# xiph/LPCNet

Measured on AMD Instinct MI355X. Metric: 16 kHz samples/sec & concurrent real-time streams, 1/2/4/8 MI355X, higher is better.
Workload: dtype f32; 1 GPU; 2048 concurrent streams (each with its own feature file) per GPU x 25 frames (4000 samples) per step, fp32 weights, register-resident block-sparse GRU-A, bit-exact (PARITY) arithmetic; eight streams per CU as two groups of four half a step apart (BASELINE config 2's 1024 streams fill half of these stream slots: `also.config2_1024_streams`); arithmetic=parity, gru_a_blocks=1382, gru_a_densities=0.05,0.05,0.2 (benchmark model), gru_a_items_per_lane=30, streams_per_gpu=2048, streams_per_workgroup=8

## Files before the change

include/lpcnet.h:

```cpp
#ifndef LPCNET_H_
#define LPCNET_H_

#ifdef __cplusplus
extern "C" {
#endif

#ifndef LPCNET_EXPORT
# if defined(__GNUC__)
#  define LPCNET_EXPORT __attribute__ ((visibility ("default")))
# else
#  define LPCNET_EXPORT
# endif
#endif

#define NB_FEATURES 20
#define NB_TOTAL_FEATURES 36
#define LPCNET_COMPRESSED_SIZE 8
#define LPCNET_PACKET_SAMPLES (4*160)
#define LPCNET_FRAME_SIZE (160)

typedef struct LPCNetState LPCNetState;
typedef struct LPCNetDecState LPCNetDecState;

LPCNET_EXPORT int lpcnet_decoder_get_size(void);
// ... 7 lines not shown
LPCNET_EXPORT int lpcnet_init(LPCNetState *st);
LPCNET_EXPORT LPCNetState *lpcnet_create(void);
LPCNET_EXPORT void lpcnet_destroy(LPCNetState *st);
LPCNET_EXPORT void lpcnet_synthesize(LPCNetState *st, const float *features, short *output, int N);
LPCNET_EXPORT int lpcnet_load_model(LPCNetState *st, const unsigned char *data, int len);

#define LPCNET_HIP_STATE_BYTES 8724

LPCNET_EXPORT void lpcnet_reset_signal(LPCNetState *lpcnet);
LPCNET_EXPORT void run_frame_network(LPCNetState *lpcnet, float *gru_a_condition, float *gru_b_condition,
                                     float *lpc, const float *features);
LPCNET_EXPORT void run_frame_network_deferred(LPCNetState *lpcnet, const float *features);
LPCNET_EXPORT void run_frame_network_flush(LPCNetState *lpcnet);
LPCNET_EXPORT void lpcnet_synthesize_tail_impl(LPCNetState *lpcnet, short *output, int N, int preload);
LPCNET_EXPORT void lpcnet_synthesize_impl(LPCNetState *lpcnet, const float *features, short *output, int N,
                                          int preload);

LPCNET_EXPORT const char *lpcnet_hip_last_error(void);
#define LPCNET_HIP_E_NODEVICE (-2)
#define LPCNET_HIP_E_DEVICE   (-3)
#define LPCNET_HIP_E_ARG      (-4)
#define LPCNET_HIP_E_MODEL    (-5)
LPCNET_EXPORT int lpcnet_hip_status(void);
LPCNET_EXPORT void lpcnet_hip_clear_error(void);
LPCNET_EXPORT int lpcnet_hip_model_status(const LPCNetState *st, int clear);
LPCNET_EXPORT int lpcnet_hip_dispatch_stats(unsigned long long *out3, int reset);
LPCNET_EXPORT const char *lpcnet_hip_build_info(void);
LPCNET_EXPORT void lpcnet_hip_set_codebooks(const float *cb1, const float *cb2, const float *cb3, const float *cb_diff4);
LPCNET_EXPORT int lpcnet_hip_set_default_model(const unsigned char *data, int len);
LPCNET_EXPORT int lpcnet_hip_decoder_load_model(LPCNetDecState *st, const unsigned char *data, int len);
LPCNET_EXPORT int lpcnet_hip_set_device(int device);
LPCNET_EXPORT int lpcnet_hip_check_model(const unsigned char *data, int len, int *info);
LPCNET_EXPORT int lpcnet_hip_x3_image_info(const unsigned char *data, int len, int *desc, int *rows, int *selftest);
LPCNET_EXPORT void lpcnet_hip_shutdown(void);

#ifdef __cplusplus
}
#endif
#endif
```

lpcnet_amd/api.py:

```python
from __future__ import annotations

import ctypes as C
import os

import numpy as np

_HERE = os.path.dirname(os.path.abspath(__file__))
LIB_PATH = os.environ.get("LPCNET_HIP_LIB") or os.path.join(_HERE, "liblpcnet_hip.so")

NB_FEATURES = 20
NB_TOTAL_FEATURES = 36
LPCNET_FRAME_SIZE = 160
LPCNET_COMPRESSED_SIZE = 8
LPCNET_PACKET_SAMPLES = 640

_f32p = np.ctypeslib.ndpointer(np.float32, flags="C_CONTIGUOUS")
_i16p = np.ctypeslib.ndpointer(np.int16, flags="C_CONTIGUOUS")
_u8p = np.ctypeslib.ndpointer(np.uint8, flags="C_CONTIGUOUS")

_lib = None


class LPCNetError(RuntimeError):
    pass
# ... 114 lines not shown
    L.lpcnet_batch_plc_enable.argtypes = [vp, C.c_int]
    L.lpcnet_batch_plc_flavour.argtypes = [vp]
    L.lpcnet_batch_plc_reset.argtypes = [vp, C.c_int, C.c_int]
    L.lpcnet_batch_plc_step.argtypes = [vp, _i16p, _u8p]
    L.lpcnet_batch_plc_step_device.argtypes = [vp, vp, _u8p, vp]
    L.lpcnet_batch_plc_step_device_shard.argtypes = [vp, C.c_int, vp, _u8p, vp]
    L.lpcnet_batch_plc_fec_add.argtypes = [vp, C.c_int, vp]
    L.lpcnet_batch_plc_fec_clear.argtypes = [vp, C.c_int]
    L.lpcnet_batch_plc_fec_feed.argtypes = [vp, vp, vp, vp, vp, vp]
    L.lpcnet_batch_plc_fec_feed_device.argtypes = [vp, vp, vp, vp, vp, vp, vp]
    L.lpcnet_batch_plc_fec_feed_device_shard.argtypes = [vp, C.c_int, vp, vp, vp, vp, vp, vp]
    L.lpcnet_hip_plc_fec_feed_plan.argtypes = [C.c_int, vp, vp, vp, vp, vp, vp]
    L.lpcnet_batch_get_plc_state.argtypes = [vp, C.c_int, vp]
    L.lpcnet_batch_set_plc_state.argtypes = [vp, C.c_int, vp]
    L.lpcnet_batch_plc_burg.argtypes = [vp, _f32p, _f32p]
    L.lpcnet_batch_plc_pred.argtypes = [vp, _f32p, _f32p]
    L.lpcnet_hip_plc_plan.argtypes = [C.c_int, C.c_int, vp, _u8p, vp, vp]
    L.lpcnet_hip_plc_model_info.argtypes = [C.c_char_p, C.c_int, C.POINTER(C.c_int)]
    L.lpcnet_batch_encode.argtypes = [vp, _i16p, _u8p, C.c_int]
    L.lpcnet_batch_encode_device.argtypes = [vp, vp, vp, C.c_int, vp]
    L.lpcnet_batch_encode_device_shard.argtypes = [vp, C.c_int, vp, vp, C.c_int, vp]
    L.lpcnet_batch_compute_features.argtypes = [vp, _i16p, _f32p, C.c_int, C.c_int]
    L.lpcnet_batch_compute_features_device.argtypes = [vp, vp, vp, C.c_int, C.c_int, vp]
    L.lpcnet_batch_encoder_enable.argtypes = [vp, C.c_int]
    L.lpcnet_batch_get_encoder_vq_mem.argtypes = [vp, C.c_int, _f32p]
    L.lpcnet_batch_set_encoder_vq_mem.argtypes = [vp, C.c_int, _f32p]
    L.lpcnet_batch_export_state.argtypes = [vp, C.c_int, vp]
    L.lpcnet_batch_import_state.argtypes = [vp, C.c_int, vp]
    L.lpcnet_batch_set_streams_per_workgroup.argtypes = [vp, C.c_int]
    L.lpcnet_batch_get_streams_per_workgroup.argtypes = [vp]
    L.lpcnet_batch_set_twelve_waves.argtypes = [vp, C.c_int]
    L.lpcnet_batch_get_twelve_waves.argtypes = [vp]
    L.lpcnet_hip_x3_image_info.argtypes = [C.c_char_p, C.c_int, C.POINTER(C.c_int), C.POINTER(C.c_int), C.POINTER(C.c_int)]
    L.lpcnet_batch_tune.argtypes = [vp]
    L.lpcnet_batch_enable_timing.argtypes = [vp, C.c_int]
    L.lpcnet_batch_last_timing.argtypes = [vp, C.POINTER(C.c_float), C.POINTER(C.c_float)]
    L.lpcnet_batch_last_error.restype = C.c_char_p
    L.lpcnet_batch_run_tail.argtypes = [vp, _f32p, _f32p, _f32p, _i16p, C.c_int, C.c_int]
    L.lpcnet_batch_run_frames.argtypes = [vp, _f32p, C.c_int, vp, vp, vp, C.c_int]
    L.lpcnet_batch_state_size.restype = C.c_int
    L.lpcnet_batch_get_raw_state.argtypes = [vp, C.c_int, vp]
    L.lpcnet_batch_set_raw_state.argtypes = [vp, C.c_int, vp]
    L.lpcnet_batch_debug_trace.argtypes = [vp, C.c_int, vp]
    L.lpcnet_batch_profile.argtypes = [vp, vp]
    _u32p = np.ctypeslib.ndpointer(np.uint32, flags="C_CONTIGUOUS")
    L.lpcnet_hip_arith_identities_device.argtypes = [_f32p, _f32p, _u32p, _u32p, _u32p, _u32p, C.c_int]
    L.lpcnet_hip_quant_sweep_device.argtypes = [C.POINTER(C.c_ulonglong)]
    L.lpcnet_hip_status.restype = C.c_int
    L.lpcnet_hip_clear_error.restype = None
    L.lpcnet_hip_model_status.argtypes = [vp, C.c_int]
    L.lpcnet_hip_build_info.restype = C.c_char_p
    L.lpcnet_hip_dispatch_stats.argtypes = [C.POINTER(C.c_ulonglong), C.c_int]
    _lib = L
    return L


def check_model(blob: bytes):
    info = (C.c_int * 6)()
    rc = load_library().lpcnet_hip_check_model(blob, len(blob), info)
    return rc, list(info)


def plc_model_info(blob: bytes):
    info = (C.c_int * 7)()
    if load_library().lpcnet_hip_plc_model_info(blob, len(blob), info) != 0:
        raise LPCNetError("plc_model_info: " + last_error())
    return dict(zip(("present", "servable", "d1", "g1", "g2", "nb1", "nb2"), list(info)))


def x3_image_info(blob: bytes):
    desc, rows, st = (C.c_int * (12 * 5 * 4))(), (C.c_int * (12 * 5 * 64))(), C.c_int(-1)
    have = load_library().lpcnet_hip_x3_image_info(blob, len(blob), desc, rows, C.byref(st))
    return have, np.array(desc, np.int32).reshape(12, 5, 4), np.array(rows, np.int32).reshape(12, 5, 64), st.value


def last_error() -> str:
    return load_library().lpcnet_hip_last_error().decode()


def status() -> int:
    return load_library().lpcnet_hip_status()


def clear_error() -> None:
    load_library().lpcnet_hip_clear_error()


def build_info() -> dict:
    txt = load_library().lpcnet_hip_build_info().decode()
    return dict(kv.split("=", 1) for kv in txt.split())


def dispatch_stats(reset=False):
    out = (C.c_ulonglong * 3)()
    load_library().lpcnet_hip_dispatch_stats(out, 1 if reset else 0)
    return int(out[0]), int(out[1]), int(out[2])


def quant_sweep():
    out = (C.c_ulonglong * 3)()
    rc = load_library().lpcnet_hip_quant_sweep_device(out)
    if rc:
        raise LPCNetError(f"lpcnet_hip_quant_sweep_device failed ({rc}): " + last_error())
    return int(out[0]), int(out[1]), int(out[2])


def arith_identities(a: np.ndarray, b: np.ndarray):
    a = np.ascontiguousarray(a, np.float32); b = np.ascontiguousarray(b, np.float32)
# ... 447 lines not shown
```

lpcnet_amd/csrc/api.c:

```c
#include <pthread.h>
#include <math.h>
#include <stddef.h>
#include <stdio.h>
#include <stdlib.h>
#include <string.h>
#include "lpcnet.h"
#include "lpcnet_batch.h"
#include "lpcnet_engine.h"

#define LPCN_MAGIC 0x4C50434Eu

#define MAX_FEATURE_BUFFER_SIZE 4

struct LPCNetState {
    uint32_t magic;
    int32_t model_id;
    lpcn_stream_state s;
    float gru_a_condition[LPCN_ROWS_A];
    float gru_b_condition[LPCN_ROWS_B];
    float feature_buffer[NB_FEATURES * MAX_FEATURE_BUFFER_SIZE];
    int32_t feature_buffer_fill;
};

_Static_assert(sizeof(struct LPCNetState) == LPCNET_HIP_STATE_BYTES, "include/lpcnet.h: LPCNET_HIP_STATE_BYTES is stale");
// ... 1497 lines not shown
        if (pf < 0) st = 100;
        else if (pf == 0) {
            f.pk_b_w = m.pk_b_w; f.pk_b_wq = m.pk_b_wq; f.pk_b_start = m.pk_b_start; f.pk_b_blk = m.pk_b_blk;
            const int sf = lpcn_model_selftest(&f);
            if (sf) st = 100 + sf;
            f.pk_b_w = NULL; f.pk_b_wq = NULL; f.pk_b_start = NULL; f.pk_b_blk = NULL;
            lpcn_model_release(&f);
        }
    }
    if (!st && !m.is_int8) {
        lpcn_model_host f;
        if (lpcn_model_pack_x2(&m, &f) == 0) {
            f.pk_b_w = m.pk_b_w; f.pk_b_start = m.pk_b_start; f.pk_b_blk = m.pk_b_blk;
            const int sf = lpcn_model_selftest(&f);
            if (sf) st = 200 + sf;
            f.pk_b_w = NULL; f.pk_b_start = NULL; f.pk_b_blk = NULL;
            lpcn_model_release(&f);
        }
    }
    if (!st) {
        lpcn_x3_image im;
        if (lpcn_model_pack_x3(&m, &im) == 0) {
            const int sf = lpcn_x3_image_selftest(&m, &im);
            if (sf) st = 300 + sf;
            lpcn_x3_image_release(&im);
        }
    }
    if (info) { info[0] = m.is_int8; info[1] = m.nb_a; info[2] = m.nb_b; info[3] = m.nw; info[4] = m.nb_b_padded; info[5] = st; }
    lpcn_model_release(&m);
    if (st) { set_err("internal error: device packing inconsistent with blob"); return -1; }
    return 0;
}

int lpcnet_hip_x3_image_info(const unsigned char *data, int len, int *desc, int *rows, int *selftest)
{
    lpcn_model_host m;
    lpcn_x3_image im;
    if (lpcn_model_parse(&m, data, len) != 0) { set_err("malformed or incomplete DNNw weight blob"); return -1; }
    const int have = lpcn_model_pack_x3(&m, &im) == 0;
    if (have) {
        if (selftest) *selftest = lpcn_x3_image_selftest(&m, &im);
        for (int w = 0; w < LPCN_X3_WAVES; w++)
            for (int k = 0; k <= LPCN_X3_SEGS; k++) {
                int *d = desc ? desc + (w * (1 + LPCN_X3_SEGS) + k) * 4 : NULL;
                if (d) { d[0] = im.kind[w][k]; d[1] = im.first[w][k]; d[2] = im.count[w][k]; d[3] = im.skip[w][k]; }
                if (rows) memcpy(rows + (w * (1 + LPCN_X3_SEGS) + k) * 64, im.row[w][k], sizeof(int) * 64);
            }
        lpcn_x3_image_release(&im);
    }
    lpcn_model_release(&m);
    return have;
}
```

lpcnet_amd/csrc/engine.hip:

```cpp
#include <hip/hip_runtime.h>
#include <stdio.h>
#include <stdlib.h>
#include <string.h>
#include <memory>
#include <vector>
#include "lpcnet_engine.h"
#include "lpcnet_tables_gen.h"
#include "sample_variants.h"
#include "sample_kernel.hip.h"
#include "frame_kernels.hip.h"
#include "decode_kernel.hip.h"
#include "analysis_kernels.hip.h"
#include "encode_kernels.hip.h"
#include "plc_kernels.hip.h"
#include "plc_plan.h"
#include <math.h>

static thread_local char g_err[512] = "";
extern "C" const char *lpcn_last_error(void) { return g_err; }

#define HIP_TRY(expr)                                                                         \
    do {                                                                                      \
        hipError_t _e = (expr);                                                               \
        if (_e != hipSuccess) {                                                               \
// ... 339 lines not shown
    UP(float, b_bias, m->b_bias, 2 * LPCN_ROWS_B);
    UP(float, fc_w, m->fc_w, 256 * 2 * LPCN_N_B);
    UP(float, fc_b, m->fc_b, 512);
    UP(float, fc_f, m->fc_f, 512);
    {
        std::vector<uint32_t> wh(256 * 2 * LPCN_N_B / 2);
        for (size_t i = 0; i < wh.size(); ++i) {
            const _Float16 lo = (_Float16)m->fc_w[2 * i], hi = (_Float16)m->fc_w[2 * i + 1];
            uint16_t l, h;
            memcpy(&l, &lo, 2); memcpy(&h, &hi, 2);
            wh[i] = (uint32_t)l | ((uint32_t)h << 16);
        }
        UP(uint32_t, fc_wh, wh.data(), wh.size());
    }
    UP(float, tab_tansig, lpcn_tansig, 201);
    UP(float, tab_ulaw2lin, lpcn_ulaw2lin_tab, 256);
    UP(float, tab_logit, lpcn_logit_tab, 256);
#undef UP
    a.nb_b = m->nb_b_padded;
    a.b_dense = m->b_dense;
    if (!m->is_int8 && m->b_dense && !getenv("LPCNET_HIP_NO_X2_IMAGE")) {
        lpcn_model_host mx;
        if (lpcn_model_pack_x2(m, &mx) == 0) {
            const int nwx = round_up_variant(variants_x2, mx.nw);
            mx.pk_b_w = m->pk_b_w; mx.pk_b_start = m->pk_b_start; mx.pk_b_blk = m->pk_b_blk;
            const int stx = lpcn_model_selftest(&mx);
            mx.pk_b_w = nullptr; mx.pk_b_start = nullptr; mx.pk_b_blk = nullptr;
            if (nwx && stx == 0) {
                LpcnSampleArgs &ax = e->image[IMG_X2].args;
                rc = upload_gru_a(&mx, e->image[IMG_X2], nwx);
                if (!rc) rc = upload<float>(e, &ax.emb_nat_sig, m->emb_sig, (size_t)256 * LPCN_ROWS_A);
                if (!rc) rc = upload<float>(e, &ax.emb_nat_pred, m->emb_pred, (size_t)256 * LPCN_ROWS_A);
                if (!rc) rc = upload<float>(e, &ax.emb_nat_exc, m->emb_exc, (size_t)256 * LPCN_ROWS_A);
            }
            lpcn_model_release(&mx);
            if (rc) return fail(rc);
        }
        lpcn_x3_image im;
        if (e->image[IMG_X2].present && lpcn_model_pack_x3(m, &im) == 0) {
            if (lpcn_x3_image_selftest(m, &im) == 0) {
                GruAImage &img = e->image[IMG_X3];
                LpcnSampleArgs &ax = img.args;
                ax = e->image[IMG_X2].args;
                int bound[LPCN_X3_WAVES * (1 + LPCN_X3_SEGS)], head[LPCN_X3_WAVES];
                for (int wv = 0; wv < LPCN_X3_WAVES; ++wv) {
                    int end = 0;
                    bound[wv * (1 + LPCN_X3_SEGS)] = 0;
                    for (int k = 1; k <= LPCN_X3_SEGS; ++k) {
                        if (im.kind[wv][k] != LPCN_X3_NONE) end = im.first[wv][k] + im.count[wv][k];
                        bound[wv * (1 + LPCN_X3_SEGS) + k] = end;
                    }
                    head[wv] = im.kind[wv][0] != LPCN_X3_NONE ? im.count[wv][0] : 0;
                }
                const float *dw = nullptr;
                rc = upload<float>(e, &dw, im.w, (size_t)LPCN_X3_WAVES * LPCN_X3_NW * 64 * 4);
                ax.a_w = (const float4 *)dw;
                if (!rc) rc = upload<uint8_t>(e, &ax.a_blk, im.blk, (size_t)LPCN_X3_WAVES * LPCN_X3_NW * 64);
                if (!rc) rc = upload<int>(e, &ax.a_row, &im.row[0][0][0], (size_t)LPCN_X3_WAVES * (1 + LPCN_X3_SEGS) * 64);
                if (!rc) rc = upload<int>(e, &ax.a_bound, bound, LPCN_X3_WAVES * (1 + LPCN_X3_SEGS));
                if (!rc) rc = upload<int>(e, &ax.a_head, head, LPCN_X3_WAVES);
                img.nw_variant = LPCN_X3_NW; img.present = rc == 0;
            }
            lpcn_x3_image_release(&im);
            if (rc) return fail(rc);
        }
    }
// ... 1466 lines not shown
```

lpcnet_amd/csrc/lpcnet_engine.h:

```cpp
#ifndef LPCNET_ENGINE_H
#define LPCNET_ENGINE_H

#include <stddef.h>
#include <stdint.h>

#ifdef __cplusplus
extern "C" {
#endif

#define LPCN_N_A        384
#define LPCN_N_B        16
#define LPCN_COND       128
#define LPCN_NB_FEAT    20
#define LPCN_PITCH_EMB  64
#define LPCN_FRAME_IN   (LPCN_NB_FEAT + LPCN_PITCH_EMB)
#define LPCN_LPC_ORDER  16
#define LPCN_NB_BANDS   18
#define LPCN_FRAME_SIZE 160
#define LPCN_FEATURES_DELAY 2
#define LPCN_ROWS_A     (3 * LPCN_N_A)
#define LPCN_ROWS_B     (3 * LPCN_N_B)

#define LPCN_WG_THREADS 512
#define LPCN_WAVES      8
#define LPCN_MAX_SLOTS  3
#define LPCN_EARLY_MAX  24
#define LPCN_DEAL_EH_F32 24
#define LPCN_DEAL_HW_I8 3
#define LPCN_I8_GBWA 2
#define LPCN_I8_GBWB 3
#define LPCN_DEAL_HMASK_I8 (0xFFu & ~((1u << LPCN_I8_GBWA) | (1u << LPCN_I8_GBWB)))
#define LPCN_DEAL_EH_I8 22
#define LPCN_X2_CHAIN_WAVES 4
#define LPCN_X2_P0_FIRST 4
#define LPCN_X2_NW_MAX 32
#define LPCN_X3_WAVES 12
#define LPCN_X3_THREADS (64 * LPCN_X3_WAVES)
#define LPCN_X3_CHAIN_WAVES 4
#define LPCN_X3_NW 16
#define LPCN_X3_SEGS 4
#define LPCN_X3_LW 4
#define LPCN_X3_FREE 9
#define LPCN_DEAL_EH_FAST_I8 0

#define LPCN_PLC_IN       (2 * LPCN_NB_BANDS + LPCN_NB_FEAT + 1)
#define LPCN_PLC_MAX_UNITS 512
#define LPCN_PLC_MAX_FEC   100
#define LPCN_PLC_BUF_SIZE  (LPCN_FEATURES_DELAY * LPCN_FRAME_SIZE + 80)
#define LPCN_PLC_QUEUE     (LPCN_PLC_BUF_SIZE + LPCN_FRAME_SIZE)
#define LPCN_PLC_FBUF      4
typedef struct lpcn_plc_model {
    int present;
    int d1, g1, g2;
    int nb1, nb2;
    const float *dense1_w, *dense1_b;
    const float *gru1_w, *gru1_rec, *gru1_bias;
    const int *gru1_idx;
    const float *gru2_w, *gru2_rec, *gru2_bias;
    const int *gru2_idx;
    const float *out_w, *out_b;
} lpcn_plc_model;

typedef struct lpcn_model_host {
    int is_int8;
    int b_dense;
    int nb_a, nb_b;
    int nw;
    int nb_b_padded;
    float lpc_gamma;

    const float *emb_sig, *emb_pred, *emb_exc;
    const float *a_dense_w, *a_dense_b;
    const float *b_dense_w, *b_dense_b;
    const float *conv1_w, *conv1_b, *conv2_w, *conv2_b;
    const float *pitch_emb;
    const float *dense1_w, *dense1_b, *dense2_w, *dense2_b;
    const float *fc_w, *fc_b, *fc_f;
    const float *a_bias, *a_diag;
    const float *a_w; const int *a_idx;
    const float *b_bias;
    const float *b_w; const int *b_idx;
    const float *b_rec;

    float   *pk_a_w;
    int32_t *pk_a_wq;
    int32_t *pk_b_wq;
    uint8_t *pk_a_blk;
    int32_t *pk_a_row;
    int32_t  pk_a_bound[LPCN_WAVES][LPCN_MAX_SLOTS + 1];
    int32_t  pk_a_allh[LPCN_WAVES][LPCN_MAX_SLOTS];
    int32_t  pk_a_head[LPCN_WAVES];
    float   *pk_b_w;
    int32_t *pk_b_start;
    uint8_t *pk_b_blk;
    float   *pk_emb[3];
    lpcn_plc_model plc;
} lpcn_model_host;

enum { LPCN_X3_NONE = 0, LPCN_X3_WHOLE = 1, LPCN_X3_HEAD = 2, LPCN_X3_TAIL = 3 };
typedef struct lpcn_x3_image {
    float   *w;
    uint8_t *blk;
    int32_t  row[LPCN_X3_WAVES][1 + LPCN_X3_SEGS][64];
    int32_t  kind[LPCN_X3_WAVES][1 + LPCN_X3_SEGS];
    int32_t  first[LPCN_X3_WAVES][1 + LPCN_X3_SEGS];
    int32_t  count[LPCN_X3_WAVES][1 + LPCN_X3_SEGS];
    int32_t  skip[LPCN_X3_WAVES][1 + LPCN_X3_SEGS];
} lpcn_x3_image;

int  lpcn_model_parse(lpcn_model_host *m, const unsigned char *blob, int len);
void lpcn_model_release(lpcn_model_host *m);
int  lpcn_model_pack_x2(const lpcn_model_host *m, lpcn_model_host *f);
int  lpcn_model_pack_fast(const lpcn_model_host *m, lpcn_model_host *f);
int  lpcn_model_pack_x3(const lpcn_model_host *m, lpcn_x3_image *im);
void lpcn_x3_image_release(lpcn_x3_image *im);
int  lpcn_x3_image_selftest(const lpcn_model_host *m, const lpcn_x3_image *im);
int  lpcn_model_selftest(const lpcn_model_host *m);
int  lpcn_plc_servable(const lpcn_model_host *m);
void lpcn_plc_pack_rec_i8(const signed char *rec, int N, int32_t *out);

typedef struct lpcn_stream_state {
    float gru_a[LPCN_N_A];
    float gru_b[LPCN_N_B];
    float conv1_mem[2 * LPCN_FRAME_IN];
// ... 152 lines not shown
```

lpcnet_amd/csrc/model_pack.c:

```c
#include <stdio.h>
#include <stdlib.h>
#include <string.h>
#include "lpcnet_engine.h"

typedef struct { const char *name; int size; const void *data; } blob_rec;

static int blob_walk(const unsigned char *p, int len, blob_rec *out, int cap)
{
    int n = 0;
    while (len > 0) {
        int32_t h[5];
        if (len < 64) return -1;
        memcpy(h, p, sizeof(h));
        if (h[3] <= 0 || h[4] < h[3] || h[4] > len - 64) return -1;
        if (h[4] & 3) return -1;
        if (p[63] != 0) return -1;
        if (n == cap) return -1;
        out[n].name = (const char *)(p + 20);
        out[n].size = h[3];
        out[n].data = p + 64;
        n++;
        p += 64 + h[4];
        len -= 64 + h[4];
    }
// ... 103 lines not shown
                }
                if (pick < 0) { ok = 0; break; }
                d.items[pick] += slot_max[z]; d.nsl[pick]++; d.nzr[pick]++; d.zr_items[pick] += slot_max[z];
                trial[z] = pick;
            }
            if (ok) {
                long mx = 0, sum = 0;
                for (int w = 0; w < LPCN_WAVES; w++) { const long c = deal_wave_cost(dp, &d, w); if (c > mx) mx = c; sum += c; }
                if (best_max < 0 || mx < best_max || (mx == best_max && sum < best_sum)) {
                    best_max = mx; best_sum = sum;
                    memcpy(best_wave, trial, sizeof(int) * (size_t)ns);
                }
            }
            depth--;
            if (depth < 0) break;
            used[perm[depth]] = 0;
        }
        int w = perm[depth] + 1;
        while (w < LPCN_WAVES && used[w]) w++;
        if (w >= LPCN_WAVES) {
            perm[depth] = -1;
            depth--;
            if (depth < 0) break;
            used[perm[depth]] = 0;
            continue;
        }
        perm[depth] = w; used[w] = 1;
        depth++;
        if (depth < nc) perm[depth] = -1;
    }
    if (best_max < 0) return -1;
    memcpy(wave_of, best_wave, sizeof(int) * (size_t)ns);
    return 0;
}

static int pack_gru_a(lpcn_model_host *m, int for_fast)
{
    deal_params dpv, *const dp = &dpv;
    enum { NG = LPCN_ROWS_A / 8, NSLOT = NG / 8 };
    row_group g[NG];
    const int *idx = m->a_idx;
    int blk = 0;
    for (int i = 0; i < NG; i++) {
        g[i].group = i; g[i].count = *idx++; g[i].pos = idx; g[i].first_block = blk;
        idx += g[i].count; blk += g[i].count;
    }
    const char *old_i8 = getenv("LPCN_DEAL_I8_OLD");
    const int deal2 = !m->is_int8 || !(old_i8 && old_i8[0] == '1');
    {
        const char *eh = getenv("LPCN_DEAL_EH");
        dp->eh = (eh && *eh) ? atoi(eh) : (m->is_int8 ? LPCN_DEAL_EH_I8 : LPCN_DEAL_EH_F32);
        {
            const char *hw = getenv("LPCN_DEAL_HW");
            dp->hw = (hw && *hw) ? atoi(hw) : (m->is_int8 ? LPCN_DEAL_HW_I8 : LPCN_WAVES / 2);
            if (dp->hw < 2) dp->hw = 2;
            if (dp->hw > LPCN_WAVES / 2) dp->hw = LPCN_WAVES / 2;
            if (!m->is_int8) dp->hw = LPCN_WAVES / 2;
            dp->hmask = (0xFFu << dp->hw) & 0xFFu;
            const char *hm = getenv("LPCN_DEAL_HMASK");
            if (m->is_int8 && !for_fast && !(hw && *hw)) dp->hmask = LPCN_DEAL_HMASK_I8;
            if (m->is_int8 && hm && *hm) dp->hmask = (unsigned)strtoul(hm, NULL, 0) & 0xFFu;
        }
        if (for_fast == 1) {
            const char *ehf = getenv("LPCN_DEAL_EH_FAST");
            dp->eh = (ehf && *ehf) ? atoi(ehf) : LPCN_DEAL_EH_FAST_I8;
        }
// ... 143 lines not shown
        int cur = 0;
        for (int k = 0; k < LPCN_MAX_SLOTS; k++) {
            const int s = slot_at[w][k], j0 = cur;
            const int head = (k == 0) ? m->pk_a_head[w] : 0;
            m->pk_a_bound[w][k] = j0;
            m->pk_a_allh[w][k] = 1;
            if (s < 0) continue;
            int allh = 1;
            for (int q = 0; q < 8; q++) {
                const row_group *rg = &g[8 * s + q];
                if (rg->group * 8 < 2 * LPCN_N_A) allh = 0;
                for (int r = 0; r < 8; r++) {
                    int lane = 8 * q + r;
                    m->pk_a_row[(w * LPCN_MAX_SLOTS + k) * 64 + lane] = rg->group * 8 + r;
                    for (int j = 0; j < rg->count; j++) {
                        const int pos = j < head ? nw - head + j : j0 + (j - head);
                        size_t item = ((size_t)w * nw + pos) * 64 + lane;
                        if (m->is_int8) {
                            const signed char *blkq = (const signed char *)m->a_w + (size_t)(rg->first_block + j) * 32;
                            memcpy(&m->pk_a_wq[item], blkq + r * 4, 4);
                        } else {
                            const float *blkw = m->a_w + (size_t)(rg->first_block + j) * 32;
                            for (int c = 0; c < 4; c++) m->pk_a_w[item * 4 + c] = blkw[c * 8 + r];
                        }
                        m->pk_a_blk[item] = (uint8_t)(rg->pos[j] >> 2);
                    }
                }
            }
            m->pk_a_allh[w][k] = allh;
            cur += slot_max[s] - head;
        }
        m->pk_a_bound[w][LPCN_MAX_SLOTS] = cur;
    }
    if (for_fast == 2) return 0;
    const float *src[3] = {m->emb_sig, m->emb_pred, m->emb_exc};
    for (int tb = 0; tb < 3; tb++) {
        float *dst = (float *)calloc((size_t)256 * LPCN_MAX_SLOTS * LPCN_WG_THREADS, sizeof(float));
        if (!dst) return -1;
        for (int v = 0; v < 256; v++)
            for (int w = 0; w < LPCN_WAVES; w++)
                for (int lane = 0; lane < 64; lane++)
                    for (int k = 0; k < LPCN_MAX_SLOTS; k++) {
                        int r = m->pk_a_row[(w * LPCN_MAX_SLOTS + k) * 64 + lane];
                        dst[((size_t)v * LPCN_MAX_SLOTS + k) * LPCN_WG_THREADS + w * 64 + lane] = r >= 0 ? src[tb][(size_t)v * LPCN_ROWS_A + r] : 0.f;
                    }
        m->pk_emb[tb] = dst;
    }
    return 0;
}

static int pack_gru_b(lpcn_model_host *m)
{
    enum { NG = LPCN_ROWS_B / 8 };
    const size_t cap = (size_t)m->nb_b + 3 * NG + 8;
    if (m->is_int8) m->pk_b_wq = (int32_t *)calloc(8 * cap, sizeof(int32_t));
    else            m->pk_b_w = (float *)calloc(32 * cap, sizeof(float));
    m->pk_b_blk = (uint8_t *)calloc(cap, 1);
    m->pk_b_start = (int32_t *)malloc(sizeof(int32_t) * (NG + 1));
    if ((!m->pk_b_w && !m->pk_b_wq) || !m->pk_b_blk || !m->pk_b_start) return -1;
    const int *idx = m->b_idx;
    int src_blk = 0, dst = 0, dense = 1;
    for (int g = 0; g < NG; g++) {
        int cnt = *idx++;
        m->pk_b_start[g] = dst;
        if (cnt != LPCN_N_A / 4) dense = 0;
        for (int j = 0; j < cnt; j++, src_blk++, dst++) {
            if (m->is_int8) {
// ... 475 lines not shown
```

lpcnet_amd/csrc/sample_kernel.hip.h:

```cpp
#pragma once
#include <hip/hip_runtime.h>
#include <stdint.h>
#include <type_traits>
#include "lpcnet_engine.h"
#include "lpcnet_math.h"

struct LpcnSampleArgs {
    const float *emb_sig, *emb_pred, *emb_exc;
    const float4 *a_w;
    const uint8_t *a_blk;
    const int *a_row;
    const int *a_bound;
    const int *a_allh;
    const int *a_head;
    const float *a_bias1;
    const float *a_diag;
    const float *b_w;
    const int *b_start;
    const uint8_t *b_blk;
    const float *b_rec;
    const float *b_bias;
    const float *fc_w, *fc_b, *fc_f;
    const float *tab_tansig, *tab_ulaw2lin, *tab_logit;
    int nb_b;
    int b_dense;
    int n_streams, n_frames, preload, fc_advance;
    int frame_len;
    const float *cond_a;
    const float *cond_b;
    const float *lpc;
    const int *fc_base;
    short *pcm;
    long long pcm_stride;
    lpcn_stream_state *state;
    float *dbg;
    unsigned long long *prof;
    const uint32_t *fc_wh;
    int fc_f16;
    const float *emb_nat_sig, *emb_nat_pred, *emb_nat_exc;
};

#ifndef LPCN_ENABLE_PROF
#define LPCN_ENABLE_PROF 0
#endif
#define LPCN_DBG_STRIDE 1600

#include "sample_common.hip.h"
#include "quant_i8.hip.h"

namespace lpcn {

#define LPCN_PROD_BLOCKS 48
template <int S> struct Lds {
    static constexpr int HA_STRIDE = 16 * S;
    static constexpr int hA     = 0;
    static constexpr int hA_sz  = 96 * HA_STRIDE + 24 * 16;
    static constexpr int pre    = hA + hA_sz;
    static constexpr int inh    = pre + S * RA * 4;
    static constexpr int cond   = inh + S * NA * 4;
    static constexpr int abias  = cond + S * RA * 4;
    static constexpr int adiag  = abias + RA * 4;
    static constexpr int hT     = adiag + RA * 4;
    static constexpr int hB     = hT + NA * S * 4;
    static constexpr int idx    = hB + S * NB * 4;
    static constexpr int thr    = idx + S * 16;
    static constexpr int mask   = thr + S * 32;
    static constexpr int lead   = mask + S * 64;
    static constexpr int flag   = lead + S * 32;
    static constexpr int condb  = flag + 16;
    static constexpr int lpc    = condb + S * RB * 4;
    static constexpr int sig    = lpc + S * 64;
    static constexpr int pcmbuf = sig + S * 64;
// ... 1291 lines not shown
```

lpcnet_amd/csrc/sample_kernel_x2.hip.h:

```cpp
#pragma once
#include "sample_kernel.hip.h"
#include "tree_stages.h"

namespace lpcn {

#define LPCN_X2_LW 4
#define LPCN_X2_TW 0
#define LPCN_X2_S2W 7
#define LPCN_X2_S2_LEAD 2
#define LPCN_X2_HG 10

struct LdsX2 {
    static constexpr int S = 4;
    static constexpr int HA_STRIDE = 16 * S;
    static constexpr int g_hA    = 0;
    static constexpr int g_hT    = g_hA + 96 * HA_STRIDE + 24 * 16;
    static constexpr int g_prec  = g_hT + NA * S * 4;
    static constexpr int g_hB    = g_prec + NA * S * 4;
    static constexpr int g_idx   = g_hB + S * NB * 4;
    static constexpr int g_thr   = g_idx + S * 16;
    static constexpr int g_mask  = g_thr + S * 32;
    static constexpr int g_pfx   = g_mask + S * 4;
    static constexpr int g_lead  = g_mask + S * 64;
    static constexpr int g_flag  = g_lead + S * 32;
    static constexpr int g_condb = g_flag + 16;
    static constexpr int g_lpc   = g_condb + S * RB * 4;
    static constexpr int g_pcm   = g_lpc + S * 64;
    static constexpr int G_SZ    = g_pcm + S * 320;
    static constexpr int pre_ur  = 2 * G_SZ;
    static constexpr int inh     = pre_ur + 2 * NA * S * 4;
    static constexpr int abias   = inh + NA * S * 4;
    static constexpr int tansig  = abias + 2 * RA * 4;
    static constexpr int ulaw    = tansig + 816;
    static constexpr int logit   = ulaw + 1024;
    static constexpr int brec    = logit + 1024;
    static constexpr int bbias   = brec + NB * RB * 4;
    static constexpr int bstart  = bbias + 2 * RB * 4;
    static constexpr int bw      = bstart + 32;
    static constexpr int total(int nb_b) { return bw + (nb_b + 8) * 128; }
    __host__ __device__ static constexpr int ha_off(int p) { return p * HA_STRIDE + (p >> 2) * 16; }
};

typedef float tree_f4 __attribute__((ext_vector_type(4)));
struct TreeRow { tree_f4 w[NB / 4]; float bias, factor; };
__device__ __forceinline__ TreeRow tree_row_load_node(const LPCN_GLOBAL float *fc_w, const LPCN_GLOBAL float *fc_b, const LPCN_GLOBAL float *fc_f, const int node, const int chan)
{
    const auto *wp = (const LPCN_GLOBAL tree_f4 *)(fc_w + (node * 2 + chan) * NB);
    TreeRow r;
#pragma unroll
    for (int j = 0; j < NB / 4; ++j) r.w[j] = wp[j];
    r.bias = fc_b[chan * 256 + node];
    r.factor = fc_f[chan * 256 + node];
    return r;
}
template <int STAGE>
__device__ __forceinline__ TreeRow tree_row_load(const LPCN_GLOBAL float *fc_w, const LPCN_GLOBAL float *fc_b, const LPCN_GLOBAL float *fc_f, const int lane, const int prefix)
{
    return tree_row_load_node(fc_w, fc_b, fc_f, lpcn_tree_node(STAGE, lpcn_tree_lane_local(STAGE, lane), prefix), lane & 1);
}
__device__ __forceinline__ TreeRow tree_row_load_packed(const LPCN_GLOBAL float *fc_w, const LPCN_GLOBAL float *fc_b, const LPCN_GLOBAL float *fc_f, const int lane, const int prefix)
{
    return tree_row_load_node(fc_w, fc_b, fc_f, lpcn_tree_packed_node(lane, prefix), lane & 1);
}
__device__ __forceinline__ unsigned long long tree_node_ballot(const TreeRow &r, const float *h_s, const float *thr, const float *tansig)
{
    const float4 *hp = (const float4 *)h_s;
    float sum = r.bias;
#pragma unroll
    for (int j = 0; j < NB / 4; ++j) {
        const float4 hv = hp[j];
        const tree_f4 wv = r.w[j];
// ... 49 lines not shown
        const int lane = tid0 & 63, wave = tid0 >> 6;
        const size_t base = (size_t)wave * NW * 64 + lane;
        const int lane_sel = (lane & 3) * 16;
        const auto *ab = as_global(Ap->a_blk);
        const auto *aw = (const LPCN_GLOBAL float *)as_global(Ap->a_w);
#pragma unroll
        for (int j = 0; j < NW; ++j) {
            const auto *v = aw + (base + (size_t)j * 64) * 4;
            w[j] = make_float4(v[0], v[1], v[2], v[3]);
        }
#pragma unroll
        for (int j = 0; j < NW; j += 2) {
            const int p0 = ab[base + (size_t)j * 64];
            const int p1 = (j + 1 < NW) ? ab[base + (size_t)(j + 1) * 64] : 0;
            offp[j >> 1] = (uint32_t)(L::ha_off(p0) + lane_sel) | ((uint32_t)(L::ha_off(p1) + lane_sel) << 16);
        }
        const auto *ar = as_global(Ap->a_row);
#pragma unroll
        for (int k = 0; k < 3; ++k) row_reg[k] = ar[(wave * 3 + k) * 64 + lane];
    }
    int b1 = __builtin_amdgcn_readfirstlane(as_global(Ap->a_bound)[(tid0 >> 6) * 4 + 1]);
    int b2 = __builtin_amdgcn_readfirstlane(as_global(Ap->a_bound)[(tid0 >> 6) * 4 + 2]);
    int b3 = __builtin_amdgcn_readfirstlane(as_global(Ap->a_bound)[(tid0 >> 6) * 4 + 3]);
    const bool allh0 = __builtin_amdgcn_readfirstlane(as_global(Ap->a_allh)[(tid0 >> 6) * 3]) != 0;
    const LPCN_GLOBAL float *fc_w_s = as_global(Ap->fc_w), *fc_b_s = as_global(Ap->fc_b), *fc_f_s = as_global(Ap->fc_f);
    asm volatile("" : "+s"(fc_w_s), "+s"(fc_b_s), "+s"(fc_f_s));
    const LPCN_GLOBAL float *cond_a_s = as_global(Ap->cond_a);
    asm volatile("" : "+s"(cond_a_s));
    const int has_slot = __builtin_amdgcn_readfirstlane((__ballot(row_reg[0] >= 0) != 0ull ? 1 : 0) | (__ballot(row_reg[1] >= 0) != 0ull ? 2 : 0) |
                                                        (__ballot(row_reg[2] >= 0) != 0ull ? 4 : 0));
    const bool has2 = (has_slot & 4) != 0;
    const int hl = __builtin_amdgcn_readfirstlane(as_global(Ap->a_head)[tid0 >> 6]);
    const bool early_wave = hl > 0;
    const bool plain_start = __builtin_amdgcn_readfirstlane(((early_wave || __ballot(row_reg[0] >= 2 * NA) == 0ull) && __ballot(row_reg[1] >= 2 * NA || row_reg[2] >= 2 * NA) == 0ull) ? 1 : 0) != 0;

    {
        const int tid = tid0;
        stage_tables<L>(smem, Ap, tid, NB * RB);
        stage_grub_weights(smem + L::bw, Ap, tid, true);
        for (int i = tid; i < 2 * S * NA; i += LPCN_WG_THREADS) {
            const int gs = i / NA, n = i % NA, g = gs >> 2, s = gs & 3;
            const float hv0 = states[stream_of(gs)].gru_a[n];
            unsigned char *gb = smem + g * L::G_SZ;
            ((float *)(gb + L::g_hT))[n * S + s] = hv0;
            *(float *)(gb + L::g_hA + L::ha_off(n >> 2) + s * 16 + (n & 3) * 4) = hv0;
        }
        for (int i = tid; i < 2 * S * NB; i += LPCN_WG_THREADS) {
            const int gs = i / NB, g = gs >> 2, s = gs & 3;
            ((float *)(smem + g * L::G_SZ + L::g_hB))[s * NB + i % NB] = states[stream_of(gs)].gru_b[i % NB];
        }
        if (tid < 2 * S) {
            const int g = tid >> 2, s = tid & 3;
            unsigned char *gb = smem + g * L::G_SZ;
            stage_leader_record({(float *)(gb + L::g_lead), (int *)(gb + L::g_idx), nullptr, nullptr}, s, &states[stream_of(tid)]);
        }
        if (tid < 2) { int *fl = (int *)(smem + tid * L::G_SZ + L::g_flag); fl[0] = 0; fl[1] = 0; }
        if (tid < 2 * S) ((int *)(smem + (tid >> 2) * L::G_SZ + L::g_pfx))[tid & 3] = 0;
    }
    __syncthreads();

    const bool is_lw = (tid0 >> 6) == LW;
    const bool is_tw_lane = tid0 >= 64 * TW && tid0 < 64 * TW + S;
#define LPCN_LROW ((tid0 & 63) >> 4)
#define LPCN_TAP (tid0 & 15)
    float histP = is_lw ? states[stream_of(S + LPCN_LROW)].last_sig[LPCN_TAP] : 0.f;
    float histQ = is_lw ? states[stream_of(LPCN_LROW)].last_sig[LPCN_TAP] : 0.f;
    bool liveP = false, liveQ = false;
    int live_maskP = 0, live_maskQ = 0;
    int seqP = 0, seqQ = 0;
    int smpP = 0, smpQ = 0, fP = 0, fQ = 0;
    float lpc_tap = 0.f, prod_old = 0.f;

    const int T = n_frames * frame_len;
#if LPCN_ENABLE_PROF
#ifndef LPCN_PROF_MASK
#define LPCN_PROF_MASK 0xFFF
#endif
    unsigned long long *const prof = Ap->prof;
    unsigned long long pt[12] = {0, 0, 0, 0, 0, 0, 0, 0, 0, 0, 0, 0}, tprev = 0;
    const bool profiling = prof != nullptr && blockIdx.x == 0;
#define LPCN_X2_PROF(slot) do { if (((LPCN_PROF_MASK >> (slot)) & 1) && profiling) { const unsigned long long now_ = __builtin_amdgcn_s_memtime(); pt[slot] += now_ - tprev; tprev = now_; } } while (0)
    if (profiling) tprev = __builtin_amdgcn_s_memtime();
#else
#define LPCN_X2_PROF(slot) do { } while (0)
#endif
    for (int h = -1; h <= 2 * T + 1; ++h) {
        const int p = h & 1, q = p ^ 1;
        unsigned char *const gp = smem + p * L::G_SZ, *const gq = smem + q * L::G_SZ;
        const bool p_active = h >= 0 && (h >> 1) < T;
        const bool p_prev = h >= 2;
// ... 253 lines not shown
                LPCN_REMAT_V(r);
                if (r >= 0) {
                    float *c = pre_cell(r, gq);
#pragma unroll
                    for (int s = 0; s < S; ++s) c[s] = acc[s];
                }
            }
            if (p0_wave) { reduce(3, 0); if (fifth) reduce(4, 1); }
            LPCN_X2_PROF(3);
        }

        static_assert(LPCN_X2_S2W > LPCN_X2_LW && LPCN_X2_S2W < LPCN_WAVES && LPCN_TREE_FIELDS == S && LPCN_X2_S2_LEAD >= 1, "stage 2 runs on a row wave other than the leader's, one field per stream");
        const bool s2_wave = q_chain && wave == LPCN_X2_S2W;
        TreeRow sub = {};
        int pfx = 0;
        auto s2_open = [&]() __attribute__((always_inline)) {
            int t_ = tid0;
            LPCN_REMAT_V(t_);
            const uint32_t cell = lds_addr(gq + L::g_pfx) + (uint32_t)lpcn_tree_packed_field(t_ & 63) * 4u;
            do {
                asm volatile("ds_read_b32 %0, %1\n\ts_waitcnt lgkmcnt(0)" : "=v"(pfx) : "v"(cell) : "memory");
            } while (__ballot((pfx >> LPCN_TREE_TOP) != seqQ) != 0ull);
            pfx &= (1 << LPCN_TREE_TOP) - 1;
            sub = tree_row_load_packed(fc_w_s, fc_b_s, fc_f_s, t_ & 63, pfx);
        };
        const bool s2_in_items = s2_wave && p_active && b3 > 0;
        if (s2_wave && !s2_in_items) s2_open();

        if (p_active) {
            hA_cur = gp + L::g_hA;
            load_negz();
            lds_poll_until<false>(p0cnt_p, seqP * NP0);
            LPCN_X2_PROF(11);
            if (plain_start) {
                int r = LPCN_ROW(0);
                LPCN_REMAT_V(r);
                r = r < 0 ? 0 : r;
                const float *c = pre_cell(r, gp);
#pragma unroll
                for (int s = 0; s < S; ++s) acc[s] = c[s];
            } else {
#pragma unroll
            for (int k = 0; k < 3; ++k) {
                int r = LPCN_ROW(k);
                LPCN_REMAT_V(r);
                const bool live_row = r >= 0;
                r = r < 0 ? 0 : r;
                const bool candidate = r >= 2 * NA;
                const int n = candidate ? r - 2 * NA : 0;
                const float bias = sm_abias[2 * r], diag = sm_abias[2 * r + 1];
                float *c = pre_cell(r, gp);
                const bool parked = k == 0 && early_wave;
#pragma unroll
                for (int s = 0; s < S; ++s) {
                    const float bv = bias + diag * hT_p[n * S + s];
                    if (k == 0) acc[s] = (candidate && !parked) ? bv : c[s];
                    else if (candidate && live_row) c[s] = bv;
                }
            }
            }
            auto row_swap = [&](const int k_done, const int k_next) __attribute__((always_inline)) {
                int r = LPCN_ROW(k_done), r2 = LPCN_ROW(k_next);
                LPCN_REMAT_V(r);
                LPCN_REMAT_V(r2);
                if (r >= 0) {
                    float *c = pre_cell(r, gp);
#pragma unroll
// ... 29 lines not shown
                if (j + PF < NW) fetch_h(j + PF);
                if (__builtin_expect(j == nextb, 0)) {
                    if (j == b1) row_swap(0, 1);
                    if (j == b2) row_swap(1, 2);
                    if (j == s2_at) s2_open();
                    __builtin_amdgcn_s_waitcnt(0xC07F);
                    nextb = b1 > j ? b1 : (b2 > j ? b2 : NW);
                    if (s2_at > j && s2_at < nextb) nextb = s2_at;
                }
                mac(j);
                return true;
            };
            auto run_items = [&](auto self, auto jc) __attribute__((always_inline)) -> void {
                constexpr int j = decltype(jc)::value;
                if constexpr (j < NW) {
                    if (!item(j)) return;
                    self(self, std::integral_constant<int, j + 1>{});
                }
            };
            run_items(run_items, std::integral_constant<int, 0>{});
            LPCN_X2_PROF(5);
            if (b1 >= jend) {
                row_swap(0, 1);
                row_swap(1, 2);
                row_store(2);
            } else if (b2 >= jend) {
                row_swap(1, 2);
                row_store(2);
            } else {
                row_store(2);
            }
            LPCN_X2_PROF(6);
        }
        if (s2_wave) {
            int t_ = tid0;
            LPCN_REMAT_V(t_);
            const int ln = t_ & 63, f = lpcn_tree_packed_field(ln);
            const unsigned long long m = tree_node_ballot(sub, hB_q + f * NB, (const float *)(gq + L::g_thr) + f * 8 + lpcn_tree_packed_level(ln), sm_tansig) & lpcn_tree_packed_mask();
            int walks = 0;
#pragma unroll
            for (int k = 0; k < S; ++k) walks |= lpcn_tree_packed_walk(m, k) << (8 * k);
            if ((ln & (LPCN_TREE_FIELD_LANES - 1)) == 0)
                ((int *)(gq + L::g_mask))[f] = (pfx << (LPCN_TREE_LEVELS - LPCN_TREE_TOP)) | ((walks >> (8 * f)) & ((1 << (LPCN_TREE_LEVELS - LPCN_TREE_TOP)) - 1));
        }
        if (q_chain && is_lw) {
            int t_ = tid0;
            LPCN_REMAT_V(t_);
            lpc_tap = ((const float *)(gq + L::g_lpc))[t_ & 63];
            prod_old = row_shr1(histQ, 0.f) * lpc_tap;
        }
        LPCN_X2_PROF(9);
        __syncthreads();
        LPCN_X2_PROF(7);

        int tid = tid0;
        LPCN_REMAT_V(tid);
        if (p_active) {
            constexpr int NI = NA * S, NQ = NI / LPCN_WG_THREADS;
            const float *const prec_p = (const float *)(gp + L::g_prec);
            float z[NQ], rg[NQ], a[NQ], hold[NQ];
#pragma unroll
            for (int k = 0; k < NQ; ++k) {
                const int i = tid + k * LPCN_WG_THREADS;
                z[k] = sm_pre_ur[i];
                rg[k] = sm_pre_ur[NI + i];
                a[k] = prec_p[i];
// ... 46 lines not shown
            const int gs = i / LPCN_FRAME_SIZE, k = i % LPCN_FRAME_SIZE;
            const short *pb = (const short *)(smem + (gs >> 2) * L::G_SZ + L::g_pcm);
            if (gs < n_valid && k < frame_len) out[(size_t)(s0 + gs) * pstride + (size_t)(n_frames - 1) * LPCN_FRAME_SIZE + k] = pb[(gs & 3) * LPCN_FRAME_SIZE + k];
        }
    }
    {
        const int tid = tid0;
        for (int i = tid; i < 2 * S * NA; i += LPCN_WG_THREADS) {
            const int gs = i / NA, n = i % NA;
            if (gs < n_valid) states[s0 + gs].gru_a[n] = ((const float *)(smem + (gs >> 2) * L::G_SZ + L::g_hT))[n * S + (gs & 3)];
        }
        for (int i = tid; i < 2 * S * NB; i += LPCN_WG_THREADS) {
            const int gs = i / NB;
            if (gs < n_valid) states[s0 + gs].gru_b[i % NB] = ((const float *)(smem + (gs >> 2) * L::G_SZ + L::g_hB))[(gs & 3) * NB + i % NB];
        }
        if (is_lw) {
            if (LPCN_LROW < n_valid) states[s0 + LPCN_LROW].last_sig[LPCN_TAP] = histP;
            if (S + LPCN_LROW < n_valid) states[s0 + S + LPCN_LROW].last_sig[LPCN_TAP] = histQ;
        }
        if (tid < n_valid) {
            auto *st = &states[s0 + tid];
            const unsigned char *gb = smem + (tid >> 2) * L::G_SZ;
            const int *li = (const int *)(gb + L::g_lead) + (tid & 3) * 8;
            const float *lp = (const float *)(gb + L::g_lpc);
#pragma unroll
            for (int j = 0; j < LPCN_LPC_ORDER; ++j) st->lpc[j] = lp[(tid & 3) * LPCN_LPC_ORDER + j];
            st->deemph_mem = ((const float *)li)[1];
            st->last_exc = li[2];
#pragma unroll
            for (int j = 0; j < 4; ++j) st->rng[j] = (uint32_t)li[4 + j];
        }
    }
#undef LPCN_ROW
#undef LPCN_LROW
#undef LPCN_TAP
}

}
```

Baseline: 168.7 million samples/s.

## Offload parked candidate-row pre-cell init to idle chain helper waves

At pack time, candidate-gate rows (index >= 2*NA) that non-head slots would otherwise initialise in the critical path are dealt to up to two chain waves that own no such rows, ordered by their total slot work. Those helper waves write bias+diag*h into the pre-cell buffer for the other group during their slack, and waves owning such rows take the plain-start path. The helper table is uploaded alongside a parked flag per wave and staged in LDS, which adds LDS footprint and extra per-step work on the helper waves. A diagnostic x2_image_info export is also added.

```diff
diff --git a/include/lpcnet.h b/include/lpcnet.h
--- a/include/lpcnet.h
+++ b/include/lpcnet.h
@@ -63,6 +63,7 @@
 LPCNET_EXPORT int lpcnet_hip_set_device(int device);
 LPCNET_EXPORT int lpcnet_hip_check_model(const unsigned char *data, int len, int *info);
 LPCNET_EXPORT int lpcnet_hip_x3_image_info(const unsigned char *data, int len, int *desc, int *rows, int *selftest);
+LPCNET_EXPORT int lpcnet_hip_x2_image_info(const unsigned char *data, int len, int *rows, int *bounds, int *head, int *help, int *parked);
 LPCNET_EXPORT void lpcnet_hip_shutdown(void);
 
 #ifdef __cplusplus
diff --git a/lpcnet_amd/api.py b/lpcnet_amd/api.py
--- a/lpcnet_amd/api.py
+++ b/lpcnet_amd/api.py
@@ -170,6 +170,7 @@
     L.lpcnet_batch_set_twelve_waves.argtypes = [vp, C.c_int]
     L.lpcnet_batch_get_twelve_waves.argtypes = [vp]
     L.lpcnet_hip_x3_image_info.argtypes = [C.c_char_p, C.c_int, C.POINTER(C.c_int), C.POINTER(C.c_int), C.POINTER(C.c_int)]
+    L.lpcnet_hip_x2_image_info.argtypes = [C.c_char_p, C.c_int] + [C.POINTER(C.c_int)] * 5
     L.lpcnet_batch_tune.argtypes = [vp]
     L.lpcnet_batch_enable_timing.argtypes = [vp, C.c_int]
     L.lpcnet_batch_last_timing.argtypes = [vp, C.POINTER(C.c_float), C.POINTER(C.c_float)]
@@ -212,6 +213,13 @@
     return have, np.array(desc, np.int32).reshape(12, 5, 4), np.array(rows, np.int32).reshape(12, 5, 64), st.value
 
 
+def x2_image_info(blob: bytes):
+    rows, bounds, head, help_, parked = (C.c_int * (8 * 3 * 64))(), (C.c_int * 32)(), (C.c_int * 8)(), (C.c_int * (4 * 3 * 64))(), (C.c_int * 8)()
+    have = load_library().lpcnet_hip_x2_image_info(blob, len(blob), rows, bounds, head, help_, parked)
+    return (have, np.array(rows, np.int32).reshape(8, 3, 64), np.array(bounds, np.int32).reshape(8, 4), np.array(head, np.int32),
+            np.array(help_, np.int32).reshape(4, 3, 64), np.array(parked, np.int32))
+
+
 def last_error() -> str:
     return load_library().lpcnet_hip_last_error().decode()
 
diff --git a/lpcnet_amd/csrc/api.c b/lpcnet_amd/csrc/api.c
--- a/lpcnet_amd/csrc/api.c
+++ b/lpcnet_amd/csrc/api.c
@@ -1553,6 +1553,23 @@
     return 0;
 }
 
+int lpcnet_hip_x2_image_info(const unsigned char *data, int len, int *rows, int *bounds, int *head, int *help, int *parked)
+{
+    lpcn_model_host m, f;
+    if (lpcn_model_parse(&m, data, len) != 0) { set_err("malformed or incomplete DNNw weight blob"); return -1; }
+    const int have = lpcn_model_pack_x2(&m, &f) == 0;
+    if (have) {
+        if (rows) memcpy(rows, f.pk_a_row, sizeof(int) * LPCN_WAVES * LPCN_MAX_SLOTS * 64);
+        if (bounds) memcpy(bounds, f.pk_a_bound, sizeof(f.pk_a_bound));
+        if (head) memcpy(head, f.pk_a_head, sizeof(f.pk_a_head));
+        if (help) memcpy(help, f.pk_a_help, sizeof(f.pk_a_help));
+        if (parked) memcpy(parked, f.pk_a_parked, sizeof(f.pk_a_parked));
+        lpcn_model_release(&f);
+    }
+    lpcn_model_release(&m);
+    return have;
+}
+
 int lpcnet_hip_x3_image_info(const unsigned char *data, int len, int *desc, int *rows, int *selftest)
 {
     lpcn_model_host m;
diff --git a/lpcnet_amd/csrc/engine.hip b/lpcnet_amd/csrc/engine.hip
--- a/lpcnet_amd/csrc/engine.hip
+++ b/lpcnet_amd/csrc/engine.hip
@@ -395,6 +395,12 @@
                 if (!rc) rc = upload<float>(e, &ax.emb_nat_sig, m->emb_sig, (size_t)256 * LPCN_ROWS_A);
                 if (!rc) rc = upload<float>(e, &ax.emb_nat_pred, m->emb_pred, (size_t)256 * LPCN_ROWS_A);
                 if (!rc) rc = upload<float>(e, &ax.emb_nat_exc, m->emb_exc, (size_t)256 * LPCN_ROWS_A);
+                if (!rc) {
+                    int help[LPCN_X2_CHAIN_WAVES * LPCN_X2_HELP_DEPTH * 64 + LPCN_WAVES];
+                    memcpy(help, mx.pk_a_help, sizeof(mx.pk_a_help));
+                    memcpy(help + LPCN_X2_CHAIN_WAVES * LPCN_X2_HELP_DEPTH * 64, mx.pk_a_parked, sizeof(mx.pk_a_parked));
+                    rc = upload<int>(e, &ax.a_help, help, LPCN_X2_CHAIN_WAVES * LPCN_X2_HELP_DEPTH * 64 + LPCN_WAVES);
+                }
             }
             lpcn_model_release(&mx);
             if (rc) return fail(rc);
diff --git a/lpcnet_amd/csrc/lpcnet_engine.h b/lpcnet_amd/csrc/lpcnet_engine.h
--- a/lpcnet_amd/csrc/lpcnet_engine.h
+++ b/lpcnet_amd/csrc/lpcnet_engine.h
@@ -34,6 +34,8 @@
 #define LPCN_X2_CHAIN_WAVES 4
 #define LPCN_X2_P0_FIRST 4
 #define LPCN_X2_NW_MAX 32
+#define LPCN_X2_HELPERS 2
+#define LPCN_X2_HELP_DEPTH 3
 #define LPCN_X3_WAVES 12
 #define LPCN_X3_THREADS (64 * LPCN_X3_WAVES)
 #define LPCN_X3_CHAIN_WAVES 4
@@ -90,6 +92,8 @@
     int32_t  pk_a_bound[LPCN_WAVES][LPCN_MAX_SLOTS + 1];
     int32_t  pk_a_allh[LPCN_WAVES][LPCN_MAX_SLOTS];
     int32_t  pk_a_head[LPCN_WAVES];
+    int32_t  pk_a_help[LPCN_X2_CHAIN_WAVES][LPCN_X2_HELP_DEPTH][64];
+    int32_t  pk_a_parked[LPCN_WAVES];
     float   *pk_b_w;
     int32_t *pk_b_start;
     uint8_t *pk_b_blk;
diff --git a/lpcnet_amd/csrc/model_pack.c b/lpcnet_amd/csrc/model_pack.c
--- a/lpcnet_amd/csrc/model_pack.c
+++ b/lpcnet_amd/csrc/model_pack.c
@@ -159,6 +159,31 @@
     if (best_max < 0) return -1;
     memcpy(wave_of, best_wave, sizeof(int) * (size_t)ns);
     return 0;
+}
+
+static void deal_helpers(lpcn_model_host *m)
+{
+    int rows[LPCN_N_A], n = 0, owner[LPCN_WAVES], helper[LPCN_X2_CHAIN_WAVES], nh = 0;
+    for (int w = 0; w < LPCN_WAVES; w++) {
+        owner[w] = 0;
+        for (int k = 0; k < LPCN_MAX_SLOTS; k++) {
+            if (k == 0 && m->pk_a_head[w] > 0) continue;
+            for (int lane = 0; lane < 64; lane++) {
+                const int r = m->pk_a_row[(w * LPCN_MAX_SLOTS + k) * 64 + lane];
+                if (r >= 2 * LPCN_N_A) { owner[w] = 1; rows[n++] = r; }
+            }
+        }
+    }
+    for (int w = 0; w < LPCN_X2_CHAIN_WAVES; w++) {
+        if (owner[w]) continue;
+        int i = nh++;
+        while (i > 0 && m->pk_a_bound[helper[i - 1]][LPCN_MAX_SLOTS] > m->pk_a_bound[w][LPCN_MAX_SLOTS]) { helper[i] = helper[i - 1]; i--; }
+        helper[i] = w;
+    }
+    if (nh > LPCN_X2_HELPERS) nh = LPCN_X2_HELPERS;
+    if (n == 0 || nh == 0 || n > nh * 64 * LPCN_X2_HELP_DEPTH) return;
+    for (int i = 0; i < n; i++) m->pk_a_help[helper[i % nh]][(i / nh) / 64][(i / nh) % 64] = rows[i];
+    for (int w = 0; w < LPCN_WAVES; w++) m->pk_a_parked[w] = owner[w];
 }
 
 static int pack_gru_a(lpcn_model_host *m, int for_fast)
@@ -368,7 +393,9 @@
         }
         m->pk_a_bound[w][LPCN_MAX_SLOTS] = cur;
     }
-    if (for_fast == 2) return 0;
+    for (int i = 0; i < LPCN_X2_CHAIN_WAVES * LPCN_X2_HELP_DEPTH * 64; i++) (&m->pk_a_help[0][0][0])[i] = -1;
+    for (int w = 0; w < LPCN_WAVES; w++) m->pk_a_parked[w] = 0;
+    if (for_fast == 2) { deal_helpers(m); return 0; }
     const float *src[3] = {m->emb_sig, m->emb_pred, m->emb_exc};
     for (int tb = 0; tb < 3; tb++) {
         float *dst = (float *)calloc((size_t)256 * LPCN_MAX_SLOTS * LPCN_WG_THREADS, sizeof(float));
diff --git a/lpcnet_amd/csrc/sample_kernel.hip.h b/lpcnet_amd/csrc/sample_kernel.hip.h
--- a/lpcnet_amd/csrc/sample_kernel.hip.h
+++ b/lpcnet_amd/csrc/sample_kernel.hip.h
@@ -38,6 +38,7 @@
     const uint32_t *fc_wh;
     int fc_f16;
     const float *emb_nat_sig, *emb_nat_pred, *emb_nat_exc;
+    const int *a_help;
 };
 
 #ifndef LPCN_ENABLE_PROF
diff --git a/lpcnet_amd/csrc/sample_kernel_x2.hip.h b/lpcnet_amd/csrc/sample_kernel_x2.hip.h
--- a/lpcnet_amd/csrc/sample_kernel_x2.hip.h
+++ b/lpcnet_amd/csrc/sample_kernel_x2.hip.h
@@ -36,7 +36,8 @@
     static constexpr int brec    = logit + 1024;
     static constexpr int bbias   = brec + NB * RB * 4;
     static constexpr int bstart  = bbias + 2 * RB * 4;
-    static constexpr int bw      = bstart + 32;
+    static constexpr int help    = bstart + 32;
+    static constexpr int bw      = help + LPCN_X2_HELP_DEPTH * 256 * 4;
     static constexpr int total(int nb_b) { return bw + (nb_b + 8) * 128; }
     __host__ __device__ static constexpr int ha_off(int p) { return p * HA_STRIDE + (p >> 2) * 16; }
 };
@@ -152,7 +153,19 @@
     const bool has2 = (has_slot & 4) != 0;
     const int hl = __builtin_amdgcn_readfirstlane(as_global(Ap->a_head)[tid0 >> 6]);
     const bool early_wave = hl > 0;
-    const bool plain_start = __builtin_amdgcn_readfirstlane(((early_wave || __ballot(row_reg[0] >= 2 * NA) == 0ull) && __ballot(row_reg[1] >= 2 * NA || row_reg[2] >= 2 * NA) == 0ull) ? 1 : 0) != 0;
+    constexpr int HD = LPCN_X2_HELP_DEPTH;
+    static_assert(LPCN_X2_CHAIN_WAVES == 4, "the helper table in LDS is [depth][256 lanes of the chain waves]");
+    int help_n = 0;
+    if (tid0 < 64 * LPCN_X2_CHAIN_WAVES) {
+#pragma unroll
+        for (int k = 0; k < HD; ++k) if (__ballot(as_global(Ap->a_help)[((tid0 >> 6) * HD + k) * 64 + (tid0 & 63)] >= 0) != 0ull) help_n = k + 1;
+    }
+    help_n = __builtin_amdgcn_readfirstlane(help_n);
+    const bool parked_rows = __builtin_amdgcn_readfirstlane(as_global(Ap->a_help)[LPCN_X2_CHAIN_WAVES * HD * 64 + (tid0 >> 6)]) != 0;
+    const bool plain_start0 = parked_rows || __builtin_amdgcn_readfirstlane(((early_wave || __ballot(row_reg[0] >= 2 * NA) == 0ull) && __ballot(row_reg[1] >= 2 * NA || row_reg[2] >= 2 * NA) == 0ull) ? 1 : 0) != 0;
+
+    int start_bits = __builtin_amdgcn_readfirstlane((plain_start0 ? 1 : 0) | (help_n << 1));
+#define LPCN_PLAIN_START ((start_bits & 1) != 0)
 
     {
         const int tid = tid0;
@@ -176,6 +189,8 @@
         }
         if (tid < 2) { int *fl = (int *)(smem + tid * L::G_SZ + L::g_flag); fl[0] = 0; fl[1] = 0; }
         if (tid < 2 * S) ((int *)(smem + (tid >> 2) * L::G_SZ + L::g_pfx))[tid & 3] = 0;
+        for (int i = tid; i < HD * 256; i += LPCN_WG_THREADS)
+            ((int *)(smem + L::help))[i] = as_global(Ap->a_help)[(((i & 255) >> 6) * HD + (i >> 8)) * 64 + (i & 63)];
     }
     __syncthreads();
 
@@ -495,7 +510,8 @@
             load_negz();
             lds_poll_until<false>(p0cnt_p, seqP * NP0);
             LPCN_X2_PROF(11);
-            if (plain_start) {
+            LPCN_REMAT_S(start_bits);
+            if (LPCN_PLAIN_START) {
                 int r = LPCN_ROW(0);
                 LPCN_REMAT_V(r);
                 r = r < 0 ? 0 : r;
@@ -591,6 +607,24 @@
             }
             LPCN_X2_PROF(6);
         }
+        LPCN_REMAT_S(start_bits);
+        if (wave < CW && q_heads && (start_bits >> 1) > 0) {
+            int t_ = tid0;
+            LPCN_REMAT_V(t_);
+            const int *hp = (const int *)(smem + L::help) + t_;
+            const float *const hT_q = (const float *)(gq + L::g_hT);
+            const int kn = start_bits >> 1;
+#pragma unroll 1
+            for (int k = 0; k < kn; ++k, hp += 256) {
+                const int r = *hp;
+                if (r >= 0) {
+                    const int n = r - 2 * NA;
+                    const float2 bd = *(const float2 *)(sm_abias + 2 * r);
+                    const float4 hv = *(const float4 *)(hT_q + n * S);
+                    *(float4 *)(gq + L::g_prec + n * (S * 4)) = make_float4(bd.x + bd.y * hv.x, bd.x + bd.y * hv.y, bd.x + bd.y * hv.z, bd.x + bd.y * hv.w);
+                }
+            }
+        }
         if (s2_wave) {
             int t_ = tid0;
             LPCN_REMAT_V(t_);
@@ -703,6 +737,7 @@
         }
     }
 #undef LPCN_ROW
+#undef LPCN_PLAIN_START
 #undef LPCN_LROW
 #undef LPCN_TAP
 }
```

After: 165.1 million samples/s. 0.979x the previous value.
